# jonassibbesen/rpvg

Measured on AMD Instinct MI355X. Metric: read-pairs quantified/sec, higher is better.
Workload: dtype f64

## Files before the change

rpvg_amd/csrc/em_plan.hpp:

```cpp
#ifndef RPVG_EM_PLAN_HPP
#define RPVG_EM_PLAN_HPP

#include <algorithm>
#include <cstddef>
#include <cstdint>

#ifndef RPVG_PLAN_FN
#if defined(__HIPCC__)
#define RPVG_PLAN_FN __host__ __device__ inline
#else
#define RPVG_PLAN_FN inline
#endif
#endif

namespace rpvg_em {

constexpr int kEmBins = 12;
constexpr int kEmGridBin = 11;
constexpr int kEmWideBin = 10;
constexpr int kEmWorkBuckets = 32;
constexpr uint32_t kEmMidGridMax = 8;
constexpr uint32_t kEmMidGridLog2 = 16;
constexpr uint32_t kEmMidBuckets = kEmWorkBuckets - kEmMidGridLog2;
constexpr int kEmStreamedBin = 3;
constexpr size_t kEmLdsLimit = 156 * 1024;
constexpr size_t kLdsOptIn = 64 * 1024;
constexpr uint32_t kRegColsMax = 32;
constexpr uint32_t kRegisterBins[5] = {6, 4, 5, 8, 9};
constexpr uint32_t kRegisterKernelIndex = 4;

RPVG_PLAN_FN size_t emLdsBytes(uint32_t cols, uint32_t rows, uint32_t entries, int block, bool resident) {
    size_t bytes = sizeof(double) * ((1 + static_cast<size_t>(block) / 64) * cols + block / 64 + 2);
    if (resident) bytes += static_cast<size_t>(rows) * 16 + static_cast<size_t>(entries) * 8 + (static_cast<size_t>(rows) + 1 + entries) * 4 + 8;
    return (bytes + 15) & ~static_cast<size_t>(15);
}

RPVG_PLAN_FN size_t emGridLdsBytes(const uint32_t cols) { return sizeof(double) * 5 * static_cast<size_t>(cols); }

RPVG_PLAN_FN size_t emRegisterLdsBytes(const int rpl, const int cols) { return (64 * static_cast<size_t>(rpl) * cols + 2) * sizeof(double); }

struct EmBinRule {
    uint32_t use_register_kernel;
    uint64_t streamed_small_work;
    uint64_t grid_min_work;
};

RPVG_PLAN_FN int emBinOf(const EmBinRule rule, const uint32_t C, const uint32_t rows, const uint32_t entries) {
    const uint64_t work = static_cast<uint64_t>(entries) + rows;
    if (rule.grid_min_work != 0 && work >= rule.grid_min_work && emGridLdsBytes(C) <= kEmLdsLimit) return kEmGridBin;
    if (rule.use_register_kernel && C <= 16 && rows <= 256) return rows <= 64 ? 4 : rows <= 128 ? 5 : 6;
    if (rule.use_register_kernel && C <= kRegColsMax && rows <= 128) return rows <= 64 ? 8 : 9;
    if (emLdsBytes(C, rows, entries, 64, true) <= 8 * 1024) return 0;
    if (emLdsBytes(C, rows, entries, 256, true) <= 40 * 1024) return 1;
    if (emLdsBytes(C, rows, entries, 1024, true) <= 152 * 1024) return 7;
    if (emLdsBytes(C, 0, 0, 256, false) > kEmLdsLimit) return kEmWideBin;
    if (emLdsBytes(C, 0, 0, 1024, false) > kEmLdsLimit) return 2;
    return work <= rule.streamed_small_work ? 2 : 3;
}

RPVG_PLAN_FN uint32_t emWorkBucket(const uint32_t rows, const uint32_t entries) {
    uint64_t work = static_cast<uint64_t>(entries) + rows + 1;
    uint32_t lg = 0;
    while (work > 1 && lg < static_cast<uint32_t>(kEmWorkBuckets - 1)) {
        work >>= 1;
        ++lg;
    }
    return static_cast<uint32_t>(kEmWorkBuckets - 1) - lg;
}

RPVG_PLAN_FN bool emIsMidSize(const uint32_t bin, const uint32_t bucket) { return bin == static_cast<uint32_t>(kEmStreamedBin) && bucket < kEmMidBuckets; }
RPVG_PLAN_FN bool emMidGridAllowed(const uint64_t grid_min_work) { return grid_min_work > (1ull << kEmMidGridLog2); }
RPVG_PLAN_FN bool emMidGridMoves(const bool allowed, const uint32_t mid) { return allowed && mid > 0 && mid <= kEmMidGridMax; }
RPVG_PLAN_FN int emRouteOf(const int bin, const uint32_t bucket, const bool moved) {
    return moved && emIsMidSize(static_cast<uint32_t>(bin), bucket) ? kEmGridBin : bin;
}

RPVG_PLAN_FN bool emIsRegisterBin(const int bin) { return bin == 4 || bin == 5 || bin == 6 || bin == 8 || bin == 9; }
RPVG_PLAN_FN int emStatsSlot(const int bin, const bool one_register_launch) {
    return emIsRegisterBin(bin) && one_register_launch ? static_cast<int>(kRegisterKernelIndex) : bin;
}

constexpr int kEmMaxFusedDense = 4;
constexpr uint32_t kEmDenseMaxCols = 2048;
RPVG_PLAN_FN bool emDenseRule(const uint32_t columns, const uint32_t rows, const uint32_t entries) {
    if (columns > kEmDenseMaxCols || columns < 2) return false;
    const uint64_t ld = (static_cast<uint64_t>(columns) + 1) & ~1ull;
    return 8ull * rows * ld <= 12ull * entries + 20ull * rows;
}

constexpr uint32_t kLdsMapPaths = 16384;
constexpr uint32_t kFillSegmentRows = 1024;
constexpr uint64_t kFillLongRowEntries = 32;
constexpr size_t kFillLongRowLds = kFillSegmentRows * (3 * sizeof(uint32_t) + sizeof(double));
constexpr size_t kFillDenseLds = kFillSegmentRows * 2 * sizeof(uint32_t);
constexpr uint64_t kFillLongRowMinWork = 1ull << 18;
RPVG_PLAN_FN size_t emFillDenseLdsBytes(const uint32_t lds_map_paths, const uint64_t widest_ld) {
    return lds_map_paths * sizeof(int32_t) + kFillDenseLds + 4 * static_cast<size_t>(widest_ld) * sizeof(double);
}

struct EmSolveKnobs {
    EmBinRule rule = {1u, 0, 1ull << 18};
    bool no_collapse = false;
    bool no_fused_dense = false;
    bool register_copies = true;
    bool one_register_launch = true;
    bool fill_thread_rows = false;
    double grid_scale = 1.0;
    bool few_streams = false;
    bool launch_early = false;
    bool wait_sort_only = false;
    bool join_on_stream = false;
    bool collapse_debug = false;
    bool has_bound_bytes = false;
    uint64_t bound_bytes = 0;
};

RPVG_PLAN_FN bool emStorageByBound(const uint64_t rows_bound, const uint64_t entries_bound, const uint64_t budget) {
    return rows_bound * 20 + entries_bound * 12 <= budget;
}
template <typename Count>
inline void emStorageBases(const Count * rows, const Count * entries, const uint32_t P, uint64_t * row_base, uint64_t * ent_base, uint64_t * rows_total,
                           uint64_t * entries_total) {
    uint64_t r = 0, e = 0;
    for (uint32_t p = 0; p < P; ++p) {
        row_base[p] = r;
        ent_base[p] = e;
        r += rows[p];
        e += entries[p];
    }
    *rows_total = r;
    *entries_total = e;
}

constexpr size_t kGibbsOneWorkgroupLdsLimit = 160 * 1024;
RPVG_PLAN_FN size_t gibbsOneWorkgroupLds(const uint32_t columns) {
    return (sizeof(double) * (2 * static_cast<size_t>(columns) + 256 / 64 + 2) + 15) & ~static_cast<size_t>(15);
}
RPVG_PLAN_FN bool gibbsTakesGrid(const uint32_t columns, const uint32_t rows, const uint32_t entries, const uint64_t grid_min_work) {
    const bool too_wide = gibbsOneWorkgroupLds(columns) > kGibbsOneWorkgroupLdsLimit;
    const bool too_large = grid_min_work != 0 && static_cast<uint64_t>(rows) + entries >= grid_min_work;
    return too_wide || too_large;
}
RPVG_PLAN_FN bool gibbsGridPossible(const uint32_t max_cols, const uint64_t max_cluster_work, const uint64_t grid_min_work) {
    return gibbsOneWorkgroupLds(max_cols) > kGibbsOneWorkgroupLdsLimit || (grid_min_work != 0 && max_cluster_work >= grid_min_work);
}

struct EmSolveShape {
    uint32_t P = 0, items_bound = 0, max_cols = 0, max_cluster_paths = 0;
    uint64_t max_cluster_work = 0, rows_capacity = 0;
    unsigned long long wide_capacity = 0;
    uint32_t cus = 0;
    int side_streams = 6;
    int hardware_queues = 4;
    bool collapse_wanted = false;
};
constexpr int kEmSideStreams = 6;
constexpr uint32_t kEmCollapseMaxProblems = (1u << 20) - 2;
constexpr uint64_t kEmCollapseMaxRows = 0x7fffffffull;

struct EmFillPlan {
    uint32_t fill_grid = 0;
    uint32_t dense_grid = 0;
    uint32_t lds_map_paths = 0;
    bool long_row_scratch = false;
    size_t fill_lds = 0;
};
inline EmFillPlan planEmFill(const EmSolveShape & s, const EmSolveKnobs & knobs) {
    EmFillPlan f;
    f.fill_grid = std::min<uint32_t>(s.items_bound, s.cus * 8);
    f.dense_grid = std::min<uint32_t>(s.items_bound, s.cus * 4);
    f.lds_map_paths = (std::min<uint32_t>(s.max_cluster_paths, kLdsMapPaths) + 3) & ~3u;
    f.long_row_scratch = !knobs.fill_thread_rows && s.max_cluster_work >= kFillLongRowMinWork;
    f.fill_lds = f.lds_map_paths * sizeof(int32_t) + (f.long_row_scratch ? kFillLongRowLds : 0);
    return f;
}

enum class EmVariant : uint8_t {
    kSparse64Resident, kSparse256Resident, kSparse1024Resident, kSparse256Streamed, kSparse1024Streamed, kSparseWide,
    kRegisterBins,
    kRegister1x16, kRegister2x16, kRegister4x16, kRegister1x32, kRegister2x32
};
constexpr int kEmMainStream = -1;
struct EmLaunch {
    uint32_t bin;
    EmVariant variant;
    uint32_t grid;
    size_t lds;
// ... 78 lines not shown
```

rpvg_amd/csrc/em_sparse.hip:

```cpp

#include "common.hpp"

#include "em_block.hpp"

#include <algorithm>
#include <memory>
#include <numeric>

using namespace rpvg_hip_detail;

namespace {

constexpr double kMinEmAbundance = 1e-8;
constexpr uint32_t kMinEmConvIts = 10;
static_assert(kEmBins == RPVG_HIP_EM_KERNELS, "a statistics slot per size bin (em_plan.hpp)");

struct EmQueues {
    uint32_t histogram[kEmBins * kEmWorkBuckets];
    uint32_t bucket_cursor[kEmBins * kEmWorkBuckets];
    uint32_t bin_start[kEmBins];
    uint32_t bin_count[kEmBins];
    uint32_t bin_cursor[kEmBins];
    uint32_t pad;
    unsigned long long wide_cursor;
    unsigned long long wide_overflow;
};


struct FillArgs {
    uint32_t num_problems;
    const uint32_t * num_problems_dev;
    uint32_t num_items;
    const uint32_t * num_items_dev;
    const uint64_t * seg_first;
    const uint32_t * item_problem;
    const uint32_t * prob_cluster;
    const uint32_t * col_path;
    const uint64_t * cluster_row_off;
    const uint64_t * cluster_path_off;
    const uint64_t * row_ent_off;
    const uint32_t * ent_path;
    const double * ent_prob;
    const double * row_count;
    const double * row_noise;
    EmProblemsView problems;
    uint32_t * seg_rows;
    uint32_t * seg_entries;
    double * seg_zero_mass;
    double * seg_total_mass;
    uint32_t * kept_entries;
    uint32_t * prob_bucket;
    EmQueues * queues;
    EmBinRule rule;
    uint32_t lds_map_paths;
    uint32_t long_row_scratch;
    uint32_t num_fused;
    EmFusedDense fused[kEmMaxFusedDense];
};

__device__ inline bool fillLongRows(const FillArgs & args, const uint32_t k) {
    const uint64_t c0 = args.cluster_row_off[k], c1 = args.cluster_row_off[k + 1];
    return args.long_row_scratch && args.row_ent_off[c1] - args.row_ent_off[c0] >= kFillLongRowEntries * (c1 - c0);
}

template <bool WRITE>
__global__ __launch_bounds__(256) void fillSegmentsKernel(const FillArgs args) {
    constexpr int BLOCK = 256;
    extern __shared__ __attribute__((aligned(16))) int32_t lds_map[];
    __shared__ uint32_t scratch[2 * (BLOCK / 64)];
    __shared__ double dscratch[BLOCK / 64];
    const uint32_t num_items = args.num_items_dev ? *args.num_items_dev : args.num_items;
    uint32_t mapped_problem = UINT32_MAX;
    for (uint32_t item = blockIdx.x; item < num_items; item += gridDim.x) {
        const uint32_t p = args.item_problem[item];
        if (WRITE) {
            bool fused = false;
            for (uint32_t f = 0; f < args.num_fused; ++f) fused = fused || args.fused[f].problem == p;
            if (fused) continue;
        }
        const uint32_t segment = static_cast<uint32_t>(item - args.seg_first[p]);
        const uint32_t k = args.prob_cluster[p];
        const uint32_t n_paths = static_cast<uint32_t>(args.cluster_path_off[k + 1] - args.cluster_path_off[k]);
        const uint32_t * cols = args.col_path + args.problems.col_off[p];
        const uint32_t n_cols = args.problems.paths(p);
        const bool use_map = n_paths <= args.lds_map_paths;
        const bool identity = n_cols == n_paths;
// ... 377 lines not shown
    __syncthreads();
    const uint32_t moved = moved_cells;
    auto cellCount = [&](const uint32_t c) -> uint32_t {
        if (c >= kCells) return 0u;
        const uint32_t bin = c / kEmWorkBuckets, bucket = c % kEmWorkBuckets;
        if (bucket < moved && bin == kEmStreamedBin) return 0u;
        if (bucket < moved && bin == kEmGridBin) return queues->histogram[c] + queues->histogram[kEmStreamedBin * kEmWorkBuckets + bucket];
        return queues->histogram[c];
    };
    {
        const uint32_t c0 = 2 * threadIdx.x, c1 = c0 + 1;
        const uint32_t h0 = cellCount(c0), h1 = cellCount(c1);
        uint32_t incl = h0 + h1;
        const int lane = threadIdx.x & 63, wave = threadIdx.x >> 6;
#pragma unroll
        for (int d = 1; d < 64; d <<= 1) {
            const uint32_t up = __shfl_up(incl, d, 64);
            if (lane >= d) incl += up;
        }
        if (lane == 63) wave_total[wave] = incl;
        __syncthreads();
        uint32_t before = 0;
        for (int w = 0; w < wave; ++w) before += wave_total[w];
        const uint32_t excl = before + incl - (h0 + h1);
        if (c0 < kCells) start[c0] = excl;
        if (c1 < kCells) start[c1] = excl + h0;
        if (threadIdx.x == 255) start[kCells] = before + incl;
    }
    __syncthreads();
    if (blockIdx.x == 0 && threadIdx.x < kEmBins) {
        queues->bin_start[threadIdx.x] = start[threadIdx.x * kEmWorkBuckets];
        queues->bin_count[threadIdx.x] = start[(threadIdx.x + 1) * kEmWorkBuckets] - start[threadIdx.x * kEmWorkBuckets];
    }
    const uint32_t p = blockIdx.x * blockDim.x + threadIdx.x;
    if (p >= P) return;
    uint32_t cell = prob_bucket[p];
    if (cell / kEmWorkBuckets == kEmStreamedBin && cell % kEmWorkBuckets < moved) cell = kEmGridBin * kEmWorkBuckets + cell % kEmWorkBuckets;
    order[start[cell] + atomicAdd(&queues->bucket_cursor[cell], 1u)] = p;
    if (cell / kEmWorkBuckets == 10) {
        const unsigned long long need = 2ull * (static_cast<unsigned long long>(col_off[p + 1] - col_off[p]) + 1);
        const unsigned long long at = atomicAdd(&queues->wide_cursor, need);
        wide_off[p] = at;
        if (at + need > wide_capacity) atomicAdd(&queues->wide_overflow, 1ull);
    }
}

struct GridDescribeArgs {
    const EmQueues * queues;
    const uint32_t * order;
    EmProblemsView problems;
    const uint32_t * kept_entries;
    EmGridProblem * out;
    uint32_t capacity;
};

__global__ __launch_bounds__(256) void emGridDescribeKernel(const GridDescribeArgs args) {
    const uint32_t i = blockIdx.x * blockDim.x + threadIdx.x;
    if (i >= args.queues->bin_count[kEmGridBin] || i >= args.capacity) return;
    const uint32_t p = args.order[args.queues->bin_start[kEmGridBin] + i];
    EmGridProblem d;
    d.problem = p;
    const EmProblemsView & v = args.problems;
    d.columns = v.paths(p) + 1;
    d.rows = v.kept_rows[p];
    d.entries = args.kept_entries[p];
    d.merged = (v.problem_merged != nullptr && v.problem_merged[p] != 0) ? 1u : 0u;
    d.pad = 0;
    d.row_base = v.row_base[p];
    d.ent_base = v.ent_base[p];
    d.col_begin = v.col_off[p];
    d.total_mass = v.total_mass[p];
    d.zero_mass = v.zero_mass[p];
    args.out[i] = d;
}


struct EmLaunchArgs {
    const uint32_t * order;
    EmQueues * queues;
    uint32_t bin;
    EmProblemsView problems;
    uint32_t max_em_its;
    uint32_t register_copies;
    double max_rel_em_conv;
    double * wide_vectors;
    const unsigned long long * wide_off;
    unsigned long long wide_capacity;
    double * abundances;
    double * noise_count;
    uint32_t * iterations;
};

template <int BLOCK>
__device__ __forceinline__ uint32_t nextProblem(const EmLaunchArgs & args, uint32_t * slot) {
    uint32_t i;
    if (BLOCK == 64) {
        i = (threadIdx.x == 0) ? atomicAdd(&args.queues->bin_cursor[args.bin], 1u) : 0u;
        i = static_cast<uint32_t>(__builtin_amdgcn_readfirstlane(static_cast<int>(i)));
    } else {
        __syncthreads();
        if (threadIdx.x == 0) *slot = atomicAdd(&args.queues->bin_cursor[args.bin], 1u);
        __syncthreads();
        i = *slot;
    }
    if (i >= args.queues->bin_count[args.bin]) return UINT32_MAX;
    return args.order[args.queues->bin_start[args.bin] + i];
}

template <int BLOCK, bool RESIDENT, bool WIDE>
__device__ __forceinline__ void emSparseProblem(const EmLaunchArgs & args, const uint32_t p, unsigned char * smem_raw) {
    const uint32_t C = args.problems.paths(p) + 1;
    if (WIDE && args.wide_off[p] + 2ull * C > args.wide_capacity) return;
    constexpr uint32_t kCopies = WIDE ? 1 : BLOCK / 64;
    double * a = WIDE ? args.wide_vectors + args.wide_off[p] : reinterpret_cast<double *>(smem_raw);
    double * t = a + C;
    double * red = WIDE ? reinterpret_cast<double *>(smem_raw) : t + static_cast<size_t>(kCopies) * C;
    double * tw = t + static_cast<size_t>(kCopies == 1 ? 0 : threadIdx.x >> 6) * C;

    const EmProblemRows csr = args.problems.mergedRows(p);
    const uint32_t n_rows = csr.rows;
    const uint32_t * off = csr.off;
    const double * cnt = csr.count;
    const double * nzv = csr.noise;
    const uint32_t * col = csr.col;
    const double * val = csr.val;
    if (RESIDENT) {
        const uint32_t n_ent = off[n_rows];
        double * l_cnt = red + (BLOCK / 64 + 2);
        double * l_nz = l_cnt + n_rows;
        double * l_val = l_nz + n_rows;
        uint32_t * l_off = reinterpret_cast<uint32_t *>(l_val + n_ent);
        uint32_t * l_col = l_off + (n_rows + 1);
        for (uint32_t r = threadIdx.x; r < n_rows; r += BLOCK) {
            l_cnt[r] = cnt[r];
            l_nz[r] = nzv[r];
        }
        for (uint32_t r = threadIdx.x; r <= n_rows; r += BLOCK) l_off[r] = off[r];
        for (uint32_t e = threadIdx.x; e < n_ent; e += BLOCK) {
            l_val[e] = val[e];
            l_col[e] = col[e];
        }
        off = l_off;
        cnt = l_cnt;
        nzv = l_nz;
        col = l_col;
        val = l_val;
    }
    const double T = args.problems.total_mass[p];
    const double Z = args.problems.zero_mass[p];
    const double eps = args.max_rel_em_conv;
    const uint32_t noise_col = C - 1;

    const double a0 = static_cast<double>(1.0f / static_cast<float>(C));
    for (uint32_t j = threadIdx.x; j < C; j += BLOCK) a[j] = a0;

    for (uint32_t j = threadIdx.x; j < kCopies * C; j += BLOCK) t[j] = 0;
    __syncthreads();

    const double inv_T = 1.0 / T;
    uint32_t iters = 0, conv = 0;
    for (uint32_t it = 0; it < args.max_em_its; ++it) {
        const double a_noise = a[noise_col];
        double tn = 0;
        for (uint32_t r = threadIdx.x; r < n_rows; r += BLOCK) {
            const uint32_t e0 = off[r], e1 = off[r + 1];
            const double nz = nzv[r];
            double s = nz * a_noise;
            for (uint32_t e = e0; e < e1; ++e) s += val[e] * a[col[e]];
            double y = __builtin_amdgcn_rcp(s);
            y = fma(fma(-s, y, 1.0), y, y);
            y = fma(fma(-s, y, 1.0), y, y);
            const double quot = cnt[r] * y;
            const double w = cnt[r] == 0.0 ? 0.0 : fma(fma(-s, quot, cnt[r]), y, quot);
            for (uint32_t e = e0; e < e1; ++e) atomicAdd(&tw[col[e]], w * val[e]);
            tn += w * nz;
        }
        tn = waveSumF64(tn);
        if ((threadIdx.x & 63) == 0 && tn != 0.0) atomicAdd(&tw[noise_col], tn);
        __syncthreads();
        int viol = 0;
        for (uint32_t j = threadIdx.x; j < C; j += BLOCK) {
            const double aj = a[j];
            double tj = t[j];
            t[j] = 0;
#pragma unroll
            for (uint32_t w = 1; w < kCopies; ++w) {
                tj += t[w * C + j];
                t[w * C + j] = 0;
            }
            const double an = (j == noise_col) ? (aj * tj + Z) * inv_T : (aj * tj) * inv_T;
            if (an >= kMinEmAbundance && fabs(an - aj) > eps * an) viol = 1;
            a[j] = an;
        }
        int any_viol;
        if (BLOCK == 64) {
            any_viol = __any(viol);
            __syncthreads();
        } else {
            any_viol = __syncthreads_or(viol);
        }
        ++iters;
        if (!any_viol) {
            if (++conv == kMinEmConvIts) break;
        } else {
            conv = 0;
        }
    }

    double low = 0;
    double * out = args.abundances + args.problems.col_off[p];
    for (uint32_t j = threadIdx.x; j < noise_col; j += BLOCK) {
        const double aj = a[j];
        if (aj < kMinEmAbundance) {
            low += aj * T;
            out[j] = 0;
        } else {
            out[j] = aj * T;
        }
    }
    low = blockReduceSum<double, BLOCK>(low, red);
    if (threadIdx.x == 0) {
        args.noise_count[p] = low + a[noise_col] * T;
        args.iterations[p] = iters;
    }
}

template <int BLOCK, bool RESIDENT, bool WIDE = false>
__global__ __launch_bounds__(BLOCK) void emSparseKernel(const EmLaunchArgs args) {
    extern __shared__ __attribute__((aligned(16))) unsigned char smem_raw[];
    __shared__ uint32_t next_slot;
    if (blockIdx.x >= args.queues->bin_count[args.bin]) return;
    for (uint32_t p = nextProblem<BLOCK>(args, &next_slot); p != UINT32_MAX; p = nextProblem<BLOCK>(args, &next_slot)) {
        emSparseProblem<BLOCK, RESIDENT, WIDE>(args, p, smem_raw);
        if (BLOCK == 64) __syncthreads();
    }
}

template <int BLOCK, bool RESIDENT, bool WIDE = false>
hipError_t launchEm(const EmLaunchArgs & args, uint32_t grid, size_t lds, hipStream_t stream) {
    if (grid == 0) return hipSuccess;
    if (lds > kLdsOptIn) {
        hipError_t e = hipFuncSetAttribute(reinterpret_cast<const void *>(&emSparseKernel<BLOCK, RESIDENT, WIDE>),
                                           hipFuncAttributeMaxDynamicSharedMemorySize, static_cast<int>(lds));
        if (e != hipSuccess) return e;
    }
    emSparseKernel<BLOCK, RESIDENT, WIDE><<<dim3(grid), dim3(BLOCK), lds, stream>>>(args);
    return hipGetLastError();
}


template <int D>
__device__ __forceinline__ double quadSwapF64(const double v) {
    constexpr int perm = (D == 1) ? 0xB1 : 0x4E;
    const int lo = __builtin_amdgcn_mov_dpp(__double2loint(v), perm, 0xF, 0xF, true);
    const int hi = __builtin_amdgcn_mov_dpp(__double2hiint(v), perm, 0xF, 0xF, true);
    return __hiloint2double(hi, lo);
// ... 172 lines not shown
}

template <int RPL, int COLS>
__device__ __forceinline__ void emRegisterBin(const EmLaunchArgs & args, const uint32_t block, double * reg_lds) {
    if (block >= args.queues->bin_count[args.bin]) return;
    for (uint32_t p = nextProblem<64>(args, nullptr); p != UINT32_MAX; p = nextProblem<64>(args, nullptr)) {
        if (RPL == 1 && COLS == 16 && args.register_copies) {
            const uint32_t n_rows = args.problems.kept_rows[p];
            if (n_rows <= 16) emRegisterProblem<1, 16, 4>(args, p, reg_lds);
            else if (n_rows <= 32) emRegisterProblem<1, 16, 2>(args, p, reg_lds);
            else emRegisterProblem<1, 16, 1>(args, p, reg_lds);
        } else {
            emRegisterProblem<RPL, COLS>(args, p, reg_lds);
        }
        __syncthreads();
    }
}

template <int RPL, int COLS>
__global__ __launch_bounds__(64) void emRegisterBinKernel(const EmLaunchArgs args) {
    extern __shared__ __attribute__((aligned(16))) double reg_lds[];
    emRegisterBin<RPL, COLS>(args, blockIdx.x, reg_lds);
}


__global__ __launch_bounds__(64) void emRegisterKernel(const EmLaunchArgs launch_args, const uint32_t variants) {
    extern __shared__ __attribute__((aligned(16))) double reg_lds[];
    EmLaunchArgs args = launch_args;
    const uint32_t variant = blockIdx.x % variants, block = blockIdx.x / variants;
    args.bin = kRegisterBins[variant];
    switch (variant) {
        case 0: emRegisterBin<4, 16>(args, block, reg_lds); break;
        case 1: emRegisterBin<1, 16>(args, block, reg_lds); break;
        case 2: emRegisterBin<2, 16>(args, block, reg_lds); break;
        case 3: emRegisterBin<1, 32>(args, block, reg_lds); break;
        default: emRegisterBin<2, 32>(args, block, reg_lds); break;
    }
}

template <int RPL, int COLS>
hipError_t launchEmRegister(const EmLaunchArgs & args, uint32_t grid, size_t lds, hipStream_t stream) {
    if (grid == 0) return hipSuccess;
    emRegisterBinKernel<RPL, COLS><<<dim3(grid), dim3(64), lds, stream>>>(args);
    return hipGetLastError();
}

hipError_t launchEmRegisterBins(const EmLaunchArgs & args, const uint32_t grid_per_bin, const bool with_32_columns, const size_t lds, hipStream_t stream) {
    if (grid_per_bin == 0) return hipSuccess;
    const uint32_t variants = with_32_columns ? 5u : 3u;
    emRegisterKernel<<<dim3(grid_per_bin * variants), dim3(64), lds, stream>>>(args, variants);
    return hipGetLastError();
}

}

namespace rpvg_hip_detail {

size_t emQueuesBytes() { return sizeof(EmQueues); }
uint32_t emFillSegmentRows() { return kFillSegmentRows; }

EmSolveKnobs emSolveKnobs() {
    static const EmSolveKnobs once = []() {
        EmSolveKnobs k;
        k.rule.use_register_kernel = RPVG_EXPERIMENT_ENV("RPVG_HIP_NO_REGISTER_EM") == nullptr ? 1u : 0u;
        k.rule.streamed_small_work = RPVG_EXPERIMENT_ENV("RPVG_HIP_EM_STREAM_SMALL") ? std::strtoull(RPVG_EXPERIMENT_ENV("RPVG_HIP_EM_STREAM_SMALL"), nullptr, 10) : 0;
        k.no_collapse = RPVG_EXPERIMENT_ENV("RPVG_HIP_NO_EM_COLLAPSE") != nullptr;
        const char * launches = std::getenv("RPVG_HIP_EM_REGISTER_LAUNCHES");
        k.one_register_launch = !(launches && std::atoi(launches) == 5);
        k.fill_thread_rows = RPVG_EXPERIMENT_ENV("RPVG_HIP_FILL_THREAD_ROWS") != nullptr;
        k.grid_scale = RPVG_EXPERIMENT_ENV("RPVG_HIP_EM_GRID_SCALE") ? std::atof(RPVG_EXPERIMENT_ENV("RPVG_HIP_EM_GRID_SCALE")) : 1.0;
        k.few_streams = RPVG_EXPERIMENT_ENV("RPVG_HIP_EM_FEW_STREAMS") != nullptr;
        k.launch_early = RPVG_EXPERIMENT_ENV("RPVG_HIP_EM_LAUNCH_EARLY") != nullptr;
        k.wait_sort_only = RPVG_EXPERIMENT_ENV("RPVG_HIP_EM_WAIT_SORT_ONLY") != nullptr;
        k.join_on_stream = RPVG_EXPERIMENT_ENV("RPVG_HIP_EM_JOIN_ON_STREAM") != nullptr;
        k.collapse_debug = RPVG_EXPERIMENT_ENV("RPVG_HIP_EM_COLLAPSE_DEBUG") != nullptr;
        return k;
    }();
    EmSolveKnobs k = once;
    k.rule.grid_min_work = emGridMinWork();
    k.no_collapse = k.no_collapse || RPVG_EXPERIMENT_ENV("RPVG_HIP_NO_COLLAPSE") != nullptr;
    k.no_fused_dense = std::getenv("RPVG_HIP_NO_FUSED_DENSE") != nullptr;
    const char * copies = std::getenv("RPVG_HIP_EM_COPIES");
    k.register_copies = copies ? std::atoi(copies) != 0 : true;
    const char * budget = std::getenv("RPVG_HIP_EM_BOUND_BYTES");
    k.has_bound_bytes = budget != nullptr;
    k.bound_bytes = budget ? static_cast<uint64_t>(std::atof(budget)) : 0;
    return k;
}

EmSolveShape emSolveShape(const rpvg_hip_ctx * ctx, const EmProblemList & list, const bool collapse_wanted) {
    EmSolveShape s;
    s.P = list.P_bound;
    s.items_bound = list.items_bound;
    s.max_cols = list.max_cols;
    s.max_cluster_paths = list.max_cluster_paths;
    s.max_cluster_work = list.max_cluster_work;
    s.rows_capacity = list.rows_capacity;
    s.wide_capacity = list.wide_capacity;
    s.cus = static_cast<uint32_t>(ctx->props.multiProcessorCount);
    s.side_streams = ctx->aux_count;
    s.hardware_queues = hardwareQueues();
    s.collapse_wanted = collapse_wanted;
    return s;
}

}

namespace {

static_assert(kEmSideStreams == rpvg_hip_ctx::kAuxStreams && kEmCollapseMaxProblems + 2 == kCollapseMaxMatrices, "em_plan.hpp restates these");

struct EmCountBuffers {
    DeviceBuffer<uint32_t> * seg_rows, * seg_entries;
    DeviceBuffer<double> * seg_zero, * seg_total;
};

int queueEmCount(rpvg_hip_ctx * ctx, const rpvg_hip_batch * batch, const EmProblemList & list, const EmOutputs & out, const EmProblemsView & view,
                 const EmCountBuffers & buffers, const EmBinRule rule, EmQueues * queues, uint32_t * prob_bucket, const EmFillPlan & plan, FillArgs & fa) {
    hipStream_t st = ctx->stream;
    RPVG_HIP_CHECK(buffers.seg_rows->alloc(list.items_bound));
    RPVG_HIP_CHECK(buffers.seg_entries->alloc(list.items_bound));
    RPVG_HIP_CHECK(buffers.seg_zero->alloc(list.items_bound));
    RPVG_HIP_CHECK(buffers.seg_total->alloc(list.items_bound));
    fa = FillArgs{};
    fa.num_problems = list.P_bound;
    fa.num_problems_dev = list.d_num_problems;
    fa.num_items = list.items_bound;
    fa.num_items_dev = list.d_num_items;
    fa.seg_first = list.d_seg_first;
    fa.item_problem = list.d_item_problem;
    fa.prob_cluster = list.d_cluster;
    fa.col_path = list.d_col_path;
    fa.cluster_row_off = batch->cluster_row_off.ptr;
    fa.cluster_path_off = batch->cluster_path_off.ptr;
    fa.row_ent_off = batch->row_ent_off.ptr;
    fa.ent_path = batch->ent_path.ptr;
    fa.ent_prob = batch->ent_prob.ptr;
    fa.row_count = batch->row_count.ptr;
    fa.row_noise = batch->row_noise.ptr;
    fa.problems = view;
    fa.seg_rows = buffers.seg_rows->ptr;
    fa.seg_entries = buffers.seg_entries->ptr;
    fa.seg_zero_mass = buffers.seg_zero->ptr;
    fa.seg_total_mass = buffers.seg_total->ptr;
    fa.kept_entries = out.d_kept_entries;
    fa.prob_bucket = prob_bucket;
    fa.queues = queues;
    fa.rule = rule;
    fa.lds_map_paths = plan.lds_map_paths;
    fa.long_row_scratch = plan.long_row_scratch ? 1u : 0u;
    fa.num_fused = 0;
    RPVG_HIP_CHECK(launchFillSegments<false>(fa, plan, st));
    fillOffsetsKernel<<<dim3((list.P_bound + 255) / 256), dim3(256), 0, st>>>(fa);
    return RPVG_HIP_OK;
}

int lookForFusedDense(rpvg_hip_ctx * ctx, const uint32_t P, EmSolveWork & work, FillArgs & fa) {
    hipStream_t st = ctx->stream;
    DeviceBuffer<DenseCandidates> d_candidates;
    DenseCandidates * h_candidates = nullptr;
    RPVG_HIP_CHECK(d_candidates.alloc(1));
    if (pinnedAlloc(reinterpret_cast<void **>(&h_candidates), sizeof(DenseCandidates)) != hipSuccess) {
        setError("rpvg_hip_em_solve: out of page-locked host memory");
        return RPVG_HIP_ERR_ALLOC;
    }
    struct PinnedGuard {
// ... 175 lines not shown
int queueEmGridAndJoin(rpvg_hip_ctx * ctx, const uint32_t P, const EmProblemsView & view, const EmOutputs & out, const EmSolveWork & work,
                       const EmSolveKnobs & knobs, EmGridLook * look, const uint32_t max_em_its, const double max_rel_em_conv) {
    hipStream_t st = ctx->stream;
    if (look) {
        RPVG_HIP_CHECK(waitEvent(look->described));
        const uint32_t n_grid = std::min<uint32_t>(*look->h_count, P);
        if (n_grid > 0) {
            std::vector<EmGridProblem> grid_problems(n_grid);
            RPVG_HIP_CHECK(hipMemcpyAsync(grid_problems.data(), look->d_problems.ptr, sizeof(EmGridProblem) * n_grid, hipMemcpyDeviceToHost, st));
            RPVG_HIP_CHECK(waitStream(st));
            EmGridStorage storage;
            storage.problems = view;
            storage.abundances = out.d_abundances;
            storage.noise_count = out.d_noise_count;
            storage.iterations = out.d_iterations;
            storage.fused = work.fused;
            storage.num_fused = work.num_fused;
            const int rc = runEmGridProblems(ctx, st, grid_problems.data(), n_grid, storage, max_em_its, max_rel_em_conv);
            if (rc != RPVG_HIP_OK) return rc;
        }
    }
    RPVG_HIP_CHECK(knobs.join_on_stream ? ctx->joinAux() : ctx->joinAuxOnHost());
    return RPVG_HIP_OK;
}

int dumpEmCollapse(rpvg_hip_ctx * ctx, const EmProblemList & list, const EmSolveWork & work) {
    const CsrCollapseWork * cw = static_cast<const CsrCollapseWork *>(work.collapse.get());
    const uint32_t P = list.P_bound;
    uint32_t info[6] = {0}, merged = 0, problems = P, counts[3] = {0};
    RPVG_HIP_CHECK(waitStream(ctx->stream));
    RPVG_HIP_CHECK(hipMemcpy(info, cw->info.ptr, sizeof(info), hipMemcpyDeviceToHost));
    RPVG_HIP_CHECK(hipMemcpy(&merged, cw->problem_merged.ptr + P, sizeof(merged), hipMemcpyDeviceToHost));
    if (list.d_num_problems) RPVG_HIP_CHECK(hipMemcpy(&problems, list.d_num_problems, sizeof(problems), hipMemcpyDeviceToHost));
    {
        const uint64_t mark_words = (list.rows_capacity + 31) / 32;
        RPVG_HIP_CHECK(hipMemcpy(counts, cw->info.ptr + 6 + 2 + 2 * static_cast<uint64_t>(P) + 1 + mark_words, sizeof(counts), hipMemcpyDeviceToHost));
    }
    std::fprintf(stderr, "[em collapse] marked rows %u forward pairs %u (equal up to rounding %u, apart %u) around pairs %u\n", counts[0], counts[1], info[4], info[5], counts[2]);
    std::fprintf(stderr, "[em collapse] problems %u (bound %u) row slots %llu: replayed %u whole %u active rows %u rows replaced %u problems merged %u\n",
                 problems, P, static_cast<unsigned long long>(list.rows_capacity), info[0], info[2], info[3], info[1], merged);
    return RPVG_HIP_OK;
}

}

namespace rpvg_hip_detail {

int queueEmSolve(rpvg_hip_ctx * ctx, const rpvg_hip_batch * batch, const EmProblemList & list, const uint32_t max_em_its,
                 const double max_rel_em_conv, const EmOutputs & out, EmSolveWork & work, const double collapse_precision) {
    hipStream_t st = ctx->stream;
    const uint32_t P = list.P_bound;
    const EmSolveKnobs knobs = emSolveKnobs();
    const EmSolvePlan plan = planEmSolve(emSolveShape(ctx, list, collapse_precision > 0), knobs);
    std::unique_ptr<HostScope> stage_scope(new HostScope("em_solve: allocations + fill queued"));
    int span = -1;
    int rc = queueEmFill(ctx, batch, list, out, work, knobs, plan.fill, plan.fused_look, span);
    if (rc != RPVG_HIP_OK) return rc;
    RPVG_REQUIRE(!plan.collapse_too_large,
                 "EM solve with a row collapse: %llu row slots in %u problems exceed what one solve can collapse (2^31 - 1 rows, 2^20 - 2 problems): split the problem list",
                 static_cast<unsigned long long>(list.rows_capacity), P);
    if (plan.collapse) {
        RPVG_HIP_CHECK(hipEventCreateWithFlags(&work.filled, hipEventDisableTiming));
        RPVG_HIP_CHECK(hipEventRecord(work.filled, st));
    }
    emOrderKernel<<<dim3((P + 255) / 256), dim3(256), 0, st>>>(P, list.d_num_problems, work.d_bucket.ptr, list.d_col_off, queuesOf(work), work.d_order.ptr,
                                                              work.d_wide_off.ptr, list.wide_capacity, plan.mid_grid_allowed ? 1u : 0u);
    RPVG_HIP_CHECK(hipGetLastError());
    ctx->spanEnd(span);
    ctx->stats.build_launches += 1;

    EmProblemsView view = work.view(list, out);
    if (plan.collapse) {
        rc = queueEmCollapse(ctx, list, plan, knobs, collapse_precision, work, view, stage_scope);
        if (rc != RPVG_HIP_OK) return rc;
    }

    EmLaunchArgs args;
    args.order = work.d_order.ptr;
    args.queues = queuesOf(work);
    args.bin = 0;
    args.problems = view;
    args.max_em_its = max_em_its;
    args.register_copies = knobs.register_copies ? 1u : 0u;
    args.max_rel_em_conv = max_rel_em_conv;
    args.wide_vectors = work.d_wide_vectors.ptr;
    args.wide_off = work.d_wide_off.ptr;
    args.wide_capacity = list.wide_capacity;
    args.abundances = out.d_abundances;
    args.noise_count = out.d_noise_count;
    args.iterations = out.d_iterations;

    EmGridLook look;
    if (plan.grid_possible) {
        rc = queueEmGridLook(ctx, P, view, out, work, look);
        if (rc != RPVG_HIP_OK) return rc;
    }
    span = ctx->spanBegin(FAM_EM_SPARSE);
    rc = queueEmLaunches(ctx, plan, args);
    if (rc != RPVG_HIP_OK) return rc;
    rc = queueEmGridAndJoin(ctx, P, view, out, work, knobs, plan.grid_possible ? &look : nullptr, max_em_its, max_rel_em_conv);
    if (rc != RPVG_HIP_OK) return rc;
    ctx->spanEnd(span);
    if (plan.collapse && knobs.collapse_debug) return dumpEmCollapse(ctx, list, work);
    return RPVG_HIP_OK;
}

void accountEmSolve(rpvg_hip_ctx * ctx, const uint32_t P, const uint64_t * col_off, const uint32_t * kept_rows, const uint32_t * kept_entries,
                    const uint32_t * iterations) {
    const EmSolveKnobs knobs = emSolveKnobs();
    const EmBinRule rule = knobs.rule;
    double bin_bytes[kEmBins] = {};
    uint64_t bin_its[kEmBins] = {}, bin_problems[kEmBins] = {};
    uint32_t bin_slowest[kEmBins] = {};
    uint32_t mid_problems = 0;
    for (uint32_t p = 0; p < P; ++p) {
        const uint32_t C = static_cast<uint32_t>(col_off[p + 1] - col_off[p]) + 1;
        if (emIsMidSize(static_cast<uint32_t>(emBinOf(rule, C, kept_rows[p], kept_entries[p])), emWorkBucket(kept_rows[p], kept_entries[p]))) ++mid_problems;
    }
    const bool mid_moved = emMidGridMoves(emMidGridAllowed(rule.grid_min_work), mid_problems);
    for (uint32_t p = 0; p < P; ++p) {
        const uint32_t C = static_cast<uint32_t>(col_off[p + 1] - col_off[p]) + 1;
        const int b = emRouteOf(emBinOf(rule, C, kept_rows[p], kept_entries[p]), emWorkBucket(kept_rows[p], kept_entries[p]), mid_moved);
        if (b == kEmGridBin && emGridDenseRoute(C, kept_rows[p], kept_entries[p])) {
            bin_problems[b] += 1;
            continue;
        }
        bin_bytes[b] += static_cast<double>(iterations[p]) * (12.0 * kept_entries[p] + 20.0 * kept_rows[p] + 16.0 * C);
        bin_its[b] += iterations[p];
        bin_problems[b] += 1;
        bin_slowest[b] = std::max(bin_slowest[b], iterations[p]);
    }
    double slot_bytes[kEmBins] = {};
    uint64_t slot_its[kEmBins] = {}, slot_problems[kEmBins] = {};
    uint32_t slot_slowest[kEmBins] = {};
    for (int b = 0; b < kEmBins; ++b) {
        const int slot = emStatsSlot(b, knobs.one_register_launch);
        slot_bytes[slot] += bin_bytes[b];
        slot_its[slot] += bin_its[b];
        slot_problems[slot] += bin_problems[b];
        slot_slowest[slot] = std::max(slot_slowest[slot], bin_slowest[b]);
    }
    for (int b = 0; b < kEmBins; ++b) {
        if (!slot_problems[b]) continue;
        rpvg_hip_em_kernel_stats & ks = ctx->stats.em_kernel[b];
        ks.launches += 1;
        ks.problems += slot_problems[b];
        ks.iterations += slot_its[b];
        ks.max_iterations += slot_slowest[b];
        ks.alg_bytes += slot_bytes[b];
        ctx->stats.em_sparse_launches += 1;
        ctx->stats.em_sparse_alg_bytes += slot_bytes[b];
        ctx->stats.em_iterations_total += slot_its[b];
    }
}

namespace {
uint64_t deviceMemoryBudget() {
    static const uint64_t budget = []() {
        size_t free_bytes = 0, total_bytes = 0;
        if (hipMemGetInfo(&free_bytes, &total_bytes) != hipSuccess) {
            (void) hipGetLastError();
            return static_cast<uint64_t>(4ull << 30);
        }
        return static_cast<uint64_t>(free_bytes) * 2 / 5;
    }();
    return budget;
// ... 145 lines not shown
```

Baseline: 2.476 billion.

## Process two rows per thread with vectorized entry prefetch in non-resident 1024-block EM

Adds a row schedule in which, for the non-resident 1024-thread EM variant, each thread handles two rows per trip. Each row's first four column indices and values are loaded with 16-byte vector loads and abundance gathers are issued before any reduction, to raise memory-level parallelism on global CSR reads. Longer rows fall back to a scalar tail loop. The risk is higher register pressure and redundant loads for short rows, and the path only covers one kernel variant; an env knob can disable it.

```diff
diff --git a/rpvg_amd/csrc/em_plan.hpp b/rpvg_amd/csrc/em_plan.hpp
--- a/rpvg_amd/csrc/em_plan.hpp
+++ b/rpvg_amd/csrc/em_plan.hpp
@@ -103,6 +103,7 @@
     bool no_collapse = false;
     bool no_fused_dense = false;
     bool register_copies = true;
+    bool rows_in_flight = true;
     bool one_register_launch = true;
     bool fill_thread_rows = false;
     double grid_scale = 1.0;
diff --git a/rpvg_amd/csrc/em_rows_plan.hpp b/rpvg_amd/csrc/em_rows_plan.hpp
--- /dev/null
+++ b/rpvg_amd/csrc/em_rows_plan.hpp
@@ -0,0 +1,40 @@
+#ifndef RPVG_EM_ROWS_PLAN_HPP
+#define RPVG_EM_ROWS_PLAN_HPP
+
+#include <cstdint>
+
+#if defined(__HIPCC__)
+#define RPVG_ROWS_FN __host__ __device__ constexpr inline
+#else
+#define RPVG_ROWS_FN constexpr inline
+#endif
+
+namespace rpvg_em_rows {
+
+struct RowSchedule {
+    uint32_t block;
+    uint32_t rows_in_flight;
+    uint32_t held_entries;
+};
+RPVG_ROWS_FN bool operator==(const RowSchedule & x, const RowSchedule & y) {
+    return x.block == y.block && x.rows_in_flight == y.rows_in_flight && x.held_entries == y.held_entries;
+}
+
+constexpr int kVariants = 5;
+RPVG_ROWS_FN RowSchedule scheduleOf(const uint32_t block, const bool resident) {
+    return !resident && block == 1024 ? RowSchedule{1024, 2, 4} : RowSchedule{block, 1, 0};
+}
+RPVG_ROWS_FN RowSchedule variantSchedule(const int variant) {
+    return variant == 0 ? scheduleOf(64, true) : variant == 1 ? scheduleOf(256, true) : variant == 2 ? scheduleOf(1024, true)
+         : variant == 3 ? scheduleOf(256, false) : scheduleOf(1024, false);
+}
+
+RPVG_ROWS_FN uint32_t rowOf(const RowSchedule & s, const uint32_t block_row, const uint32_t lane) { return block_row * s.block + lane; }
+RPVG_ROWS_FN uint32_t blockRowsOf(const RowSchedule & s, const uint32_t rows) { return (rows + s.block - 1) / s.block; }
+RPVG_ROWS_FN uint32_t fullTripsOf(const RowSchedule & s, const uint32_t rows) { return blockRowsOf(s, rows) / s.rows_in_flight; }
+RPVG_ROWS_FN uint32_t heldOf(const RowSchedule & s, const uint32_t length) { return length < s.held_entries ? length : s.held_entries; }
+RPVG_ROWS_FN bool hasTail(const RowSchedule & s, const uint32_t length) { return length > s.held_entries; }
+
+}
+
+#endif
diff --git a/rpvg_amd/csrc/em_sparse.hip b/rpvg_amd/csrc/em_sparse.hip
--- a/rpvg_amd/csrc/em_sparse.hip
+++ b/rpvg_amd/csrc/em_sparse.hip
@@ -2,6 +2,7 @@
 #include "common.hpp"
 
 #include "em_block.hpp"
+#include "em_rows_plan.hpp"
 
 #include <algorithm>
 #include <memory>
@@ -545,6 +546,7 @@
     EmProblemsView problems;
     uint32_t max_em_its;
     uint32_t register_copies;
+    uint32_t rows_in_flight;
     double max_rel_em_conv;
     double * wide_vectors;
     const unsigned long long * wide_off;
@@ -570,11 +572,115 @@
     return args.order[args.queues->bin_start[args.bin] + i];
 }
 
+__device__ __forceinline__ double emRowWeight(const double cnt, const double s) {
+    double y = __builtin_amdgcn_rcp(s);
+    y = fma(fma(-s, y, 1.0), y, y);
+    y = fma(fma(-s, y, 1.0), y, y);
+    const double quot = cnt * y;
+    return cnt == 0.0 ? 0.0 : fma(fma(-s, quot, cnt), y, quot);
+}
+
+struct __attribute__((packed, aligned(4))) EntryColumns4 {
+    uint32_t x[4];
+};
+struct __attribute__((packed, aligned(8))) EntryValues2 {
+    double x[2];
+};
+
+template <uint32_t U, uint32_t K>
+__device__ __forceinline__ void emRowsTrip(const rpvg_em_rows::RowSchedule schedule, const uint32_t first, const uint32_t n_rows, const uint32_t n_ent,
+                                           const uint32_t * off, const double * cnt, const double * nzv, const uint32_t * col, const double * val,
+                                           const double * a, double * tw, const double a_noise, double & tn) {
+    static_assert(K == 4, "four columns in one load of 16 bytes, four values in two");
+    uint32_t e0[U], len[U];
+    double nz[U], c[U];
+#pragma unroll
+    for (uint32_t u = 0; u < U; ++u) {
+        const uint32_t r = rpvg_em_rows::rowOf(schedule, first + u, threadIdx.x);
+        const bool ok = r < n_rows;
+        const uint32_t rc = ok ? r : n_rows - 1;
+        e0[u] = off[rc];
+        len[u] = ok ? off[rc + 1] - e0[u] : 0u;
+        nz[u] = nzv[rc];
+        c[u] = ok ? cnt[rc] : 0.0;
+    }
+    uint32_t cj[U][K];
+    double v[U][K];
+#pragma unroll
+    for (uint32_t u = 0; u < U; ++u) {
+        const uint32_t from = min(e0[u], n_ent - K);
+        const EntryColumns4 c4 = *reinterpret_cast<const EntryColumns4 *>(col + from);
+        const EntryValues2 v01 = *reinterpret_cast<const EntryValues2 *>(val + from), v23 = *reinterpret_cast<const EntryValues2 *>(val + from + 2);
+#pragma unroll
+        for (uint32_t k = 0; k < K; ++k) {
+            cj[u][k] = c4.x[k];
+            v[u][k] = k < 2 ? v01.x[k & 1] : v23.x[k & 1];
+        }
+        if (from != e0[u]) {
+            const uint32_t shift = e0[u] - from;
+#pragma unroll
+            for (uint32_t k = 0; k + 1 < K; ++k) {
+#pragma unroll
+                for (uint32_t j = k + 1; j < K; ++j) {
+                    if (k + shift == j) {
+                        cj[u][k] = c4.x[j];
+                        v[u][k] = j < 2 ? v01.x[j & 1] : v23.x[j & 1];
+                    }
+                }
+            }
+        }
+    }
+    double av[U][K];
+#pragma unroll
+    for (uint32_t u = 0; u < U; ++u) {
+#pragma unroll
+        for (uint32_t k = 0; k < K; ++k) av[u][k] = a[cj[u][k]];
+    }
+    double w[U];
+#pragma unroll
+    for (uint32_t u = 0; u < U; ++u) {
+        double s = nz[u] * a_noise;
+#pragma unroll
+        for (uint32_t k = 0; k < K; ++k) {
+            if (k < len[u]) s += v[u][k] * av[u][k];
+        }
+        if (rpvg_em_rows::hasTail(schedule, len[u])) {
+            for (uint32_t e = e0[u] + K; e < e0[u] + len[u]; ++e) s += val[e] * a[col[e]];
+        }
+        w[u] = emRowWeight(c[u], s);
+    }
+#pragma unroll
+    for (uint32_t u = 0; u < U; ++u) {
+#pragma unroll
+        for (uint32_t k = 0; k < K; ++k) {
+            if (k < len[u]) atomicAdd(&tw[cj[u][k]], w[u] * v[u][k]);
+        }
+        if (rpvg_em_rows::hasTail(schedule, len[u])) {
+            for (uint32_t e = e0[u] + K; e < e0[u] + len[u]; ++e) atomicAdd(&tw[col[e]], w[u] * val[e]);
+        }
+        tn += w[u] * nz[u];
+    }
+}
+
+template <uint32_t U, uint32_t K>
+__device__ __forceinline__ double emRowsInFlight(const rpvg_em_rows::RowSchedule schedule, const uint32_t n_rows, const uint32_t n_ent, const uint32_t * off,
+                                                 const double * cnt, const double * nzv, const uint32_t * col, const double * val, const double * a,
+                                                 double * tw, const double a_noise) {
+    double tn = 0;
+    const uint32_t block_rows = rpvg_em_rows::blockRowsOf(schedule, n_rows), in_trips = rpvg_em_rows::fullTripsOf(schedule, n_rows) * U;
+    for (uint32_t j = 0; j < in_trips; j += U) emRowsTrip<U, K>(schedule, j, n_rows, n_ent, off, cnt, nzv, col, val, a, tw, a_noise, tn);
+    for (uint32_t j = in_trips; j < block_rows; ++j) emRowsTrip<1, K>(schedule, j, n_rows, n_ent, off, cnt, nzv, col, val, a, tw, a_noise, tn);
+    return tn;
+}
+
 template <int BLOCK, bool RESIDENT, bool WIDE>
 __device__ __forceinline__ void emSparseProblem(const EmLaunchArgs & args, const uint32_t p, unsigned char * smem_raw) {
     const uint32_t C = args.problems.paths(p) + 1;
     if (WIDE && args.wide_off[p] + 2ull * C > args.wide_capacity) return;
     constexpr uint32_t kCopies = WIDE ? 1 : BLOCK / 64;
+    constexpr rpvg_em_rows::RowSchedule kSchedule = WIDE ? rpvg_em_rows::RowSchedule{BLOCK, 1, 0} : rpvg_em_rows::scheduleOf(BLOCK, RESIDENT);
+    static_assert(kSchedule.block == BLOCK, "the schedule of this variant (em_rows_plan.hpp)");
+    static_assert(kSchedule.rows_in_flight == 1 || !RESIDENT, "emRowsTrip loads 16 bytes at a time from global memory");
     double * a = WIDE ? args.wide_vectors + args.wide_off[p] : reinterpret_cast<double *>(smem_raw);
     double * t = a + C;
     double * red = WIDE ? reinterpret_cast<double *>(smem_raw) : t + static_cast<size_t>(kCopies) * C;
@@ -621,20 +727,21 @@
     __syncthreads();
 
     const double inv_T = 1.0 / T;
+    const uint32_t n_entries = csr.off[n_rows];
+    const bool rows_in_flight = kSchedule.rows_in_flight > 1 && args.rows_in_flight && n_rows > 0 && n_entries >= kSchedule.held_entries;
     uint32_t iters = 0, conv = 0;
     for (uint32_t it = 0; it < args.max_em_its; ++it) {
         const double a_noise = a[noise_col];
         double tn = 0;
-        for (uint32_t r = threadIdx.x; r < n_rows; r += BLOCK) {
+        if constexpr (kSchedule.rows_in_flight > 1) {
+            if (rows_in_flight) tn = emRowsInFlight<kSchedule.rows_in_flight, kSchedule.held_entries>(kSchedule, n_rows, n_entries, off, cnt, nzv, col, val, a, tw, a_noise);
+        }
+        for (uint32_t r = threadIdx.x; !rows_in_flight && r < n_rows; r += BLOCK) {
             const uint32_t e0 = off[r], e1 = off[r + 1];
             const double nz = nzv[r];
             double s = nz * a_noise;
             for (uint32_t e = e0; e < e1; ++e) s += val[e] * a[col[e]];
-            double y = __builtin_amdgcn_rcp(s);
-            y = fma(fma(-s, y, 1.0), y, y);
-            y = fma(fma(-s, y, 1.0), y, y);
-            const double quot = cnt[r] * y;
-            const double w = cnt[r] == 0.0 ? 0.0 : fma(fma(-s, quot, cnt[r]), y, quot);
+            const double w = emRowWeight(cnt[r], s);
             for (uint32_t e = e0; e < e1; ++e) atomicAdd(&tw[col[e]], w * val[e]);
             tn += w * nz;
         }
@@ -973,6 +1080,8 @@
     k.no_fused_dense = std::getenv("RPVG_HIP_NO_FUSED_DENSE") != nullptr;
     const char * copies = std::getenv("RPVG_HIP_EM_COPIES");
     k.register_copies = copies ? std::atoi(copies) != 0 : true;
+    const char * in_flight = std::getenv("RPVG_HIP_EM_ROWS_IN_FLIGHT");
+    k.rows_in_flight = in_flight ? std::atoi(in_flight) != 0 : true;
     const char * budget = std::getenv("RPVG_HIP_EM_BOUND_BYTES");
     k.has_bound_bytes = budget != nullptr;
     k.bound_bytes = budget ? static_cast<uint64_t>(std::atof(budget)) : 0;
@@ -1314,6 +1423,7 @@
     args.problems = view;
     args.max_em_its = max_em_its;
     args.register_copies = knobs.register_copies ? 1u : 0u;
+    args.rows_in_flight = knobs.rows_in_flight ? 1u : 0u;
     args.max_rel_em_conv = max_rel_em_conv;
     args.wide_vectors = work.d_wide_vectors.ptr;
     args.wide_off = work.d_wide_off.ptr;
```

After: 2.466 billion. About the same (-0.4%).
